# Giovannibriglia/ContinuousBayesianNetwork

Hardware: NVIDIA B200
Metric: posterior queries/sec (batched VE) (higher is better)
Workload: dtype f32

## Files before the change

continuousbayesiannetwork_b200/_native.py:

```python
from __future__ import annotations

import ctypes as C
import os
from typing import Dict, Sequence

PKG = os.path.dirname(os.path.abspath(__file__))
LIB_PATH = os.path.join(PKG, "libcbn_b200.so")

MAX_FAMILY_VARS = 12
MAX_CARD = 255
UNSEEN = 255
MAX_CONTRACT_DIMS = 24
MAX_CONTRACT_INPUTS = 16
MAX_GATHER_TABLES = 16
MAX_EVIDENCE_PTRS = 64
GATHER_MAX_CT = 8

OK, ERR_INVALID, ERR_CUDA, ERR_NOMEM, ERR_UNSUPPORTED = 0, -1, -2, -3, -4


class NativeLibraryMissing(ImportError):
    pass


# ... 96 lines not shown
    "cbn_cpt_from_counts": (C.c_int, [_P, _P, C.POINTER(Family), C.c_int32, C.c_longlong, _P, _P, _P]),
    "cbn_cpt_from_plan": (C.c_int, [_P, _P, _P, C.c_longlong, _P, _P, _P]),
    "cbn_cpt_from_plan_dev": (C.c_int, [_P, _P, _P, _P, _P, _P, _P]),
    "cbn_mle_from_counts": (C.c_int, [_P, _P, C.POINTER(Family), C.POINTER(_P), C.c_longlong, _P, _P, _P]),
    "cbn_get_prob_f32": (C.c_int, [_P, _P, C.POINTER(Family), C.POINTER(_P), _P, C.c_int64, C.c_int32, _P,
                                   C.c_int64, _P, _P]),
    "cbn_factor_contract": (C.c_int, [_P, C.POINTER(Contract), _P]),
    "cbn_factor_rescale": (C.c_int, [_P, _P, C.c_longlong, C.c_int32, C.c_int32, _P]),
    "cbn_ve_plan_create_gather": (C.c_int, [_P, C.c_int32, C.POINTER(C.c_int32), C.c_int32, C.POINTER(GatherTable),
                                            C.c_int32, C.c_int32, _P, C.POINTER(_P)]),
    "cbn_ve_plan_create_rows": (C.c_int, [_P, C.c_int32, C.POINTER(C.c_int32), C.c_int32, C.POINTER(RowInput), C.c_int32,
                                          C.POINTER(RowStep), C.c_int32, C.c_int32, _P, C.POINTER(_P)]),
    "cbn_ve_plan_destroy": (None, [_P]),
    "cbn_ve_plan_fuse": (C.c_int, [_P, C.POINTER(_P), C.c_int32, _P, C.POINTER(_P)]),
    "cbn_ve_plan_set_static_evidence": (C.c_int, [_P, C.c_int32]),
    "cbn_ve_plan_outputs": (C.c_int, [_P]),
    "cbn_ve_run_codes_multi": (C.c_int, [_P, _P, _P, C.c_int64, C.c_int64, C.POINTER(_P), _P]),
    "cbn_ve_run_codes": (C.c_int, [_P, _P, _P, C.c_int64, C.c_int64, _P, _P]),
    "cbn_ve_run_f32": (C.c_int, [_P, _P, C.POINTER(_P), C.POINTER(_P), C.c_int64, _P, _P]),
    "cbn_ve_run_codes_map": (C.c_int, [_P, _P, _P, C.c_int64, C.c_int64, _P, _P, _P]),
    "cbn_ve_run_f32_map": (C.c_int, [_P, _P, C.POINTER(_P), C.POINTER(_P), C.c_int64, _P, _P, _P]),
    "cbn_ve_run_codes_log_evidence": (C.c_int, [_P, _P, _P, C.c_int64, C.c_int64, _P, _P]),
    "cbn_loglik_plan_create": (C.c_int, [_P, C.POINTER(Family), C.c_int32, C.c_int32, _P, _P, C.POINTER(_P)]),
    "cbn_loglik_plan_destroy": (None, [_P]),
    "cbn_loglik_run": (C.c_int, [_P, _P, _P, C.c_int64, C.c_int64, _P, C.c_int32, _P]),
    "cbn_loglik_plan_tables": (C.c_int, [_P]),
    "cbn_factor_contract_max": (C.c_int, [_P, C.POINTER(Contract), _P, _P]),
    "cbn_mpe_plan_create": (C.c_int, [_P, C.c_int32, C.POINTER(C.c_int32), C.c_int32, C.POINTER(MpeStep), C.c_int32, _P,
                                      C.POINTER(_P)]),
    "cbn_mpe_plan_destroy": (None, [_P]),
# ... 112 lines not shown
```

continuousbayesiannetwork_b200/csrc/common.cuh:

```cuda
#pragma once
#include <cuda_runtime.h>
#include <stdint.h>
#include <stdio.h>
#include <stdarg.h>
#include <string>
#include <vector>

#include "cbn_b200.h"

struct cbn_ctx {
  int device = 0;
  int sm_count = 148;
  size_t smem_optin = 0;
  std::string err;
  cudaStream_t io_stream[2] = {nullptr, nullptr};
  cudaEvent_t io_event[2] = {nullptr, nullptr};
  void* io_dev_in[2] = {nullptr, nullptr};
  void* io_dev_out[2] = {nullptr, nullptr};
  void* io_pin_in[2] = {nullptr, nullptr};
  void* io_pin_out[2] = {nullptr, nullptr};
  size_t io_in_bytes = 0, io_out_bytes = 0;
  cudaMemPool_t pool = nullptr;
};

// ... 140 lines not shown
  asm volatile("ld.global.nc.L1::no_allocate.v8.f32 {%0,%1,%2,%3,%4,%5,%6,%7}, [%8];"
               : "=f"(v[0]), "=f"(v[1]), "=f"(v[2]), "=f"(v[3]), "=f"(v[4]), "=f"(v[5]), "=f"(v[6]), "=f"(v[7])
               : "l"(p));
}

__device__ __forceinline__ void st_f256_hint(float* p, const float* v, uint64_t pol) {
  asm volatile("st.global.L2::cache_hint.v8.f32 [%0], {%1,%2,%3,%4,%5,%6,%7,%8}, %9;" ::"l"(p), "f"(v[0]), "f"(v[1]), "f"(v[2]),
               "f"(v[3]), "f"(v[4]), "f"(v[5]), "f"(v[6]), "f"(v[7]), "l"(pol)
               : "memory");
}
__device__ __forceinline__ void ld_na_f256_hint(const float* p, float* v, uint64_t pol) {
  asm volatile("ld.global.nc.L1::no_allocate.L2::cache_hint.v8.f32 {%0,%1,%2,%3,%4,%5,%6,%7}, [%8], %9;"
               : "=f"(v[0]), "=f"(v[1]), "=f"(v[2]), "=f"(v[3]), "=f"(v[4]), "=f"(v[5]), "=f"(v[6]), "=f"(v[7])
               : "l"(p), "l"(pol));
}
__device__ __forceinline__ void bulk_g2s_hint(void* dst, const void* src, uint32_t bytes, uint64_t* bar, uint64_t pol) {
  asm volatile("cp.async.bulk.shared::cluster.global.mbarrier::complete_tx::bytes.L2::cache_hint [%0], [%1], %2, [%3], %4;" ::"r"(smem_u32(dst)),
               "l"(src), "r"(bytes), "r"(smem_u32(bar)), "l"(pol)
               : "memory");
}
```

continuousbayesiannetwork_b200/csrc/ve.cu:

```cuda
#include <stdlib.h>
#include <string.h>

#include <algorithm>
#include <new>

#include "common.cuh"

namespace {
struct ContractMagic { unsigned long long m[CBN_MAX_CONTRACT_DIMS]; int sh[CBN_MAX_CONTRACT_DIMS]; };

__device__ __forceinline__ float lse_pair(float a, float b) {
  const float NEG_INF = __int_as_float(0xff800000);
  const float hi = fmaxf(a, b), lo = fminf(a, b);
  return (hi == NEG_INF) ? NEG_INF : hi + log1pf(expf(lo - hi));
}

template <bool FAST, bool LOG, bool MAX = false>
__global__ void __launch_bounds__(256) contract_kernel(const __grid_constant__ cbn_contract d, const __grid_constant__ ContractMagic mg,
                                                       long long n_out, uint8_t* __restrict__ amax) {
  for (long long o = (long long)blockIdx.x * blockDim.x + threadIdx.x; o < n_out;
       o += (long long)gridDim.x * blockDim.x) {
    long long base[CBN_MAX_CONTRACT_INPUTS];
#pragma unroll
    for (int k = 0; k < CBN_MAX_CONTRACT_INPUTS; ++k) base[k] = 0;
// ... 328 lines not shown
  int n_out = 1;
  unsigned normalize_mask = 1;
  int log_space = 0;
  std::vector<int> ev_cards;
  std::vector<GTable> h_tables;
  int kind = 0;
  int rows_n_inputs = 0, rows_n_steps = 0, rows_temp_floats = 0, rows_flags = 0;
  void* d_row_inputs = nullptr;
  void* d_row_steps = nullptr;
  void* d_row_offsets = nullptr;
  int rows_off_ints = 0;
  size_t rows_thread_smem = 0;
  bool rows_per_thread = false;
  float* d_inter = nullptr;
  int interleaved = 0;
  unsigned char* d_blob = nullptr;
  size_t blob_bytes = 0;
  size_t desc_bytes = 0;
  int staged = 0;
  long long table_bytes = 0;
  int static_evidence = 0;
  mutable int occ[4] = {0, 0, 0, 0};
  mutable size_t occ_smem[4] = {0, 0, 0, 0};
};

namespace {
struct EvPtrs {
  const float* col[CBN_MAX_EVIDENCE_PTRS];
  const float* dom[CBN_MAX_EVIDENCE_PTRS];
  int card[CBN_MAX_EVIDENCE_PTRS];
// ... 46 lines not shown
  } else {
#pragma unroll
    for (int t = 0; t < CT; ++t) v[t] = src[t];
  }
}

template <int CT>
__device__ __forceinline__ void load_slice_l2(const float* __restrict__ src, float (&v)[CT]) {
  if constexpr (CT == 8) {
    ld_na_f256(src, v);
  } else if constexpr (CT == 4) {
    const float4 a = ld_nc_f128(reinterpret_cast<const float4*>(src));
    v[0] = a.x; v[1] = a.y; v[2] = a.z; v[3] = a.w;
  } else {
    load_slice<CT>(src, v);
  }
}

__device__ __forceinline__ void pdl_trigger() { asm volatile("griddepcontrol.launch_dependents;" ::: "memory"); }
__device__ __forceinline__ void pdl_wait() { asm volatile("griddepcontrol.wait;" ::: "memory"); }

template <int CT>
__device__ __forceinline__ void finish_rows4(float (&p)[4][CT], uint32_t bad, bool normalize, int64_t quad,
                                             int64_t n_rows, float* __restrict__ out, uint64_t st_pol = 0, bool log_space = false) {
  pdl_wait();
  if (log_space) {
#pragma unroll
    for (int r = 0; r < 4; ++r) {
      float m = p[r][0];
#pragma unroll
// ... 225 lines not shown
#pragma unroll
        for (int t = 0; t < CT; ++t) p[r][t] = lg ? p[r][t] + s : p[r][t] * s;
      }
    }
  }
  if (cur >= 0) finish_any4<CT, LOGEV>(p, bad, (outs.normalize_mask >> cur) & 1u, quad, n_rows, outs, cur, st_pol);
}

__device__ __forceinline__ void stage_blob(const unsigned char* __restrict__ blob, int blob_bytes, unsigned char* smem) {
  const uint4* src = reinterpret_cast<const uint4*>(blob);
  uint4* dst = reinterpret_cast<uint4*>(smem);
  for (int i = threadIdx.x; i < (blob_bytes >> 4); i += blockDim.x) dst[i] = __ldg(src + i);
  __syncthreads();
}

template <int CT, int NOUT, typename Loader>
__device__ __forceinline__ void gather_inter_rows4(const GTable& T, const float* __restrict__ base, const Loader& L,
                                                   int64_t quad, int64_t n_rows, const GatherOuts& outs, uint64_t st_pol = 0,
                                                   uint64_t ld_pol = 0) {
  constexpr int W = CT * NOUT;
  uint32_t i0 = 0, i1 = 0, i2 = 0, i3 = 0, any = 0, bad = 0;
  const int mode = T.flags >> GT_MODE_SHIFT;
  const int ne = T.n_ev;
  const uint32_t tm = ((quad << 2) + 4 <= n_rows) ? 0xffffffffu : ((1u << (8 * int(n_rows - (quad << 2)))) - 1u);
  if (mode == 0) {
    uint32_t acc = 0;
#pragma unroll 4
    for (int j = 0; j < ne; ++j) {
      const uint32_t w = L.load4(T.slot[j], quad) & tm;
      any |= w;
      acc += w * (uint32_t)T.stride[j];
    }
    i0 = acc & 0xffu; i1 = (acc >> 8) & 0xffu; i2 = (acc >> 16) & 0xffu; i3 = acc >> 24;
  } else if (mode == 1) {
    uint32_t accE = 0, accO = 0;
// ... 18 lines not shown
  const uint32_t lim = (uint32_t)T.n_cells - W;
  if (any & 0x80808080u) {
    const uint4 e = exact_index4(T, L, quad, lim, &bad);
    i0 = e.x; i1 = e.y; i2 = e.z; i3 = e.w;
    bad &= tm == 0xffffffffu ? 0xfu : ((1u << int(n_rows - (quad << 2))) - 1u);
  }
  i0 = min(i0, lim); i1 = min(i1, lim); i2 = min(i2, lim); i3 = min(i3, lim);
  const uint32_t idx[4] = {i0, i1, i2, i3};
  float v[4][W];
  if (T.smem_off >= 0) {
#pragma unroll
    for (int r = 0; r < 4; ++r) load_slice<W>(base + idx[r], v[r]);
  } else if (W == 8 && ld_pol) {
#pragma unroll
    for (int r = 0; r < 4; ++r) ld_na_f256_hint(base + idx[r], v[r], ld_pol);
  } else {
#pragma unroll
    for (int r = 0; r < 4; ++r) load_slice_l2<W>(base + idx[r], v[r]);
  }
#pragma unroll
  for (int o = 0; o < NOUT; ++o) {
    float p[4][CT];
#pragma unroll
    for (int r = 0; r < 4; ++r)
#pragma unroll
      for (int t = 0; t < CT; ++t) p[r][t] = v[r][o * CT + t];
    finish_rows4<CT>(p, bad, false, quad, n_rows, outs.out[o], st_pol);
  }
}

template <int CT, int NOUT>
__global__ void __launch_bounds__(GATHER_TPB) gather_inter_kernel(const unsigned char* __restrict__ blob, int blob_bytes,
                                                                  int desc_bytes, const uint8_t* __restrict__ ev, int64_t ld,
                                                                  int64_t n_rows, int early_ev, const __grid_constant__ GatherOuts outs) {
  extern __shared__ __align__(16) unsigned char smem_raw[];
  pdl_trigger();
  stage_blob(blob, blob_bytes, smem_raw);
  if (!early_ev) pdl_wait();
  const GTable& T = *reinterpret_cast<const GTable*>(smem_raw);
  const float* base = T.smem_off >= 0 ? reinterpret_cast<const float*>(smem_raw + desc_bytes) + T.smem_off : T.data;
  CodeLoader L{ev, ld};
  const int64_t nquads = (n_rows + 3) >> 2;
  for (int64_t q = int64_t(blockIdx.x) * blockDim.x + threadIdx.x; q < nquads; q += int64_t(gridDim.x) * blockDim.x)
    gather_inter_rows4<CT, NOUT>(T, base, L, q, n_rows, outs);
}

constexpr int GT_MAX_QPT = 2;
constexpr int GT_TILE_ROWS_MAX = 4 * GATHER_TPB * GT_MAX_QPT;
constexpr int GT_MAX_COLS = 16;
constexpr int GT_MAX_STAGES = 4;

struct TileCols {
  int n;
  uint8_t slot[GT_MAX_COLS];
};
template <int TILE_ROWS>
struct TileLoader {
  const unsigned char* stage;
  int64_t quad0;
  __device__ __forceinline__ uint32_t load4(int col, int64_t quad) const {
    return *reinterpret_cast<const uint32_t*>(stage + col * TILE_ROWS + (int(quad - quad0) << 2));
  }
};

template <int CT, int NOUT, int GT_QPT, bool LOGEV = false>
__global__ void __launch_bounds__(GATHER_TPB) gather_tiles_kernel(const unsigned char* __restrict__ blob, int blob_bytes,
                                                                  int desc_bytes, int n_tables, const __grid_constant__ TileCols cols,
                                                                  int n_stages, int hints, const uint8_t* __restrict__ ev, int64_t ld,
                                                                  int64_t n_rows, int early_ev, const __grid_constant__ GatherOuts outs) {
  constexpr int GT_TILE_ROWS = 4 * GATHER_TPB * GT_QPT;
  extern __shared__ __align__(128) unsigned char smem_raw[];
  __shared__ __align__(8) uint64_t full[GT_MAX_STAGES], empty[GT_MAX_STAGES];
  pdl_trigger();
  stage_blob(blob, blob_bytes, smem_raw);
  if (!early_ev) pdl_wait();
  GTable* st = reinterpret_cast<GTable*>(smem_raw);
  for (int i = threadIdx.x; i < n_tables * GATHER_MAX_TABLE_EV; i += blockDim.x) {
    GTable& T = st[i / GATHER_MAX_TABLE_EV];
    const int j = i % GATHER_MAX_TABLE_EV;
    if (j < T.n_ev) {
// ... 42 lines not shown
        if (i > 0) mbar_wait(&empty[(i - 1) % n_stages], uint32_t((i - 1) / n_stages) & 1u);
        issue(nxt);
      }
    }
    mbar_wait(&full[s], round & 1u);
    const int64_t tile = int64_t(blockIdx.x) + i * gridDim.x;
    const int64_t q0 = tile * (GT_TILE_ROWS / 4);
    TileLoader<GT_TILE_ROWS> L{stages + size_t(s) * stage_bytes, q0};
#pragma unroll 1
    for (int qq = 0; qq < GT_QPT; ++qq) {
      const int64_t q = q0 + qq * GATHER_TPB + threadIdx.x;
      if (q < nquads) {
        if constexpr (NOUT >= 2) {
          const GTable& T = st[0];
          const float* base = T.smem_off >= 0 ? pool + T.smem_off : T.data;
          gather_inter_rows4<CT, NOUT>(T, base, L, q, n_rows, outs, st_pol, ld_pol);
        } else {
          gather_rows4<CT, TileLoader<GT_TILE_ROWS>, LOGEV>(st, n_tables, pool, L, q, n_rows, outs, st_pol, ld_pol);
        }
      }
    }
    __syncwarp();
    if (lane == 0) mbar_arrive(&empty[s]);
  }
}

constexpr int gather_min_blocks(int ct) { return ct <= 2 ? 6 : (ct <= 4 ? 5 : 3); }

template <int CT, bool LOGEV = false>
__global__ void __launch_bounds__(GATHER_TPB, gather_min_blocks(LOGEV && CT == 2 ? 3 : CT)) gather_codes_kernel(
    const unsigned char* __restrict__ blob, int blob_bytes, int desc_bytes, int n_tables, const uint8_t* __restrict__ ev,
// ... 167 lines not shown
  if (rc) { cbn_ve_plan_destroy(p); return rc; }
  *out = p;
  return CBN_OK;
}

extern "C" int cbn_ve_plan_fuse(cbn_ctx* ctx, const cbn_ve_plan* const* plans, int32_t n_plans, cbn_stream stream,
                                cbn_ve_plan** out) {
  cudaStream_t cs = (cudaStream_t)stream;
  if (!ctx) return cbn_fail(nullptr, CBN_ERR_INVALID, "cbn_ve_plan_fuse: ctx is NULL");
  if (!plans || !out || n_plans < 1) return cbn_fail(ctx, CBN_ERR_INVALID, "cbn_ve_plan_fuse: bad argument");
  DeviceGuard g(ctx->device);
  cbn_ve_plan* p = new (std::nothrow) cbn_ve_plan();
  if (!p) return cbn_fail(ctx, CBN_ERR_NOMEM, "out of host memory");
  p->device = ctx->device;
  p->n_out = 0; p->normalize_mask = 0;
  for (int i = 0; i < n_plans; ++i) {
    const cbn_ve_plan* q = plans[i];
    if (!q) { delete p; return cbn_fail(ctx, CBN_ERR_INVALID, "cbn_ve_plan_fuse: plan %d is NULL", i); }
    if (q->kind != 0) { delete p; return cbn_fail(ctx, CBN_ERR_INVALID, "cbn_ve_plan_fuse: per-row plans cannot be fused"); }
    if (i == 0) { p->n_evidence = q->n_evidence; p->ev_cards = q->ev_cards; p->card_t = q->card_t; p->log_space = q->log_space; }
    if (q->ev_cards != p->ev_cards || q->card_t != p->card_t || q->log_space != p->log_space) {
      delete p;
      return cbn_fail(ctx, CBN_ERR_INVALID, "cbn_ve_plan_fuse: plans must share the evidence list, the target cardinality and the number space");
    }
    for (int o = 0; o < q->n_out; ++o) {
      if (p->n_out >= GATHER_MAX_OUT) { delete p; return cbn_fail(ctx, CBN_ERR_UNSUPPORTED, "cbn_ve_plan_fuse: at most %d targets per launch", GATHER_MAX_OUT); }
      for (const GTable& t : q->h_tables)
        if (t.out_id == o) { GTable c = t; c.out_id = p->n_out; p->h_tables.push_back(c); }
      if ((q->normalize_mask >> o) & 1u) p->normalize_mask |= 1u << p->n_out;
      p->n_out += 1;
    }
  }
  {
    const int n_out = p->n_out, ct = p->card_t, w = n_out * ct;
    bool ok = n_out >= 2 && ct >= 2 && (int)p->h_tables.size() == n_out && p->normalize_mask == 0 && ct <= GATHER_MAX_CT &&
              (w == 4 || w == 6 || w == 8);
    for (int k = 0; ok && k < n_out; ++k) {
      const GTable& t = p->h_tables[k];
      ok = (t.flags & GT_HAS_TARGET) && t.out_id == k && (k == 0 || same_index(t, p->h_tables[0])) &&
           (long long)t.n_cells * n_out <= 0x7fffffffll;
    }
    if (ok) {
      const long long n_cfg = p->h_tables[0].n_cells / ct;
      cudaError_t e = cudaMalloc((void**)&p->d_inter, size_t(n_cfg) * w * sizeof(float));
      for (int k = 0; e == cudaSuccess && k < n_out; ++k)
        e = cudaMemcpy2DAsync(p->d_inter + k * ct, size_t(w) * sizeof(float), p->h_tables[k].data, size_t(ct) * sizeof(float),
                              size_t(ct) * sizeof(float), size_t(n_cfg), cudaMemcpyDeviceToDevice, cs);
      if (e != cudaSuccess) { cbn_ve_plan_destroy(p); return cbn_fail(ctx, CBN_ERR_CUDA, "interleave: %s", cudaGetErrorString(e)); }
      GTable t = p->h_tables[0];
      t.data = p->d_inter;
      t.n_cells = (int)(n_cfg * w);
      for (int j = 0; j < t.n_ev; ++j) t.stride[j] *= n_out;
      p->h_tables.assign(1, t);
      p->interleaved = n_out;
    }
  }
  int rc = finalize_plan(ctx, p, cs);
  if (rc) { cbn_ve_plan_destroy(p); return rc; }
  *out = p;
  return CBN_OK;
}

extern "C" int cbn_ve_plan_set_static_evidence(cbn_ve_plan* plan, int32_t on) {
  if (!plan) return CBN_ERR_INVALID;
  plan->static_evidence = on ? 1 : 0;
  return CBN_OK;
}

extern "C" int cbn_ve_plan_outputs(const cbn_ve_plan* plan) { return plan ? plan->n_out : 0; }

extern "C" void cbn_ve_plan_destroy(cbn_ve_plan* p) {
  if (!p) return;
  DeviceGuard g(p->device);
  if (p->d_blob) cudaFree(p->d_blob);
// ... 54 lines not shown
int launch_f32(cbn_ctx* ctx, const cbn_ve_plan* p, const EvPtrs& evp, size_t dom_floats, int64_t n_rows, const GatherOuts& outs,
               cudaStream_t s) {
  static bool attr_set[64] = {};
  if (!attr_set[ctx->device & 63]) {
    CBN_CUDA(ctx, cudaFuncSetAttribute(gather_f32_kernel<CT>, cudaFuncAttributeMaxDynamicSharedMemorySize, 160 * 1024));
    attr_set[ctx->device & 63] = true;
  }
  size_t smem = p->blob_bytes + dom_floats * 4;
  int per_sm = (int)std::max<size_t>(1, std::min<size_t>(4, (200 * 1024) / (smem + 1024)));
  gather_f32_kernel<CT><<<gather_blocks(ctx, n_rows, per_sm), GATHER_TPB, smem, s>>>(
      p->d_blob, (int)p->blob_bytes, (int)p->desc_bytes, p->n_tables, evp, p->n_evidence, n_rows, outs);
  CBN_CHECK_LAUNCH(ctx);
  return CBN_OK;
}

template <int CT, int NOUT>
int launch_inter(cbn_ctx* ctx, const cbn_ve_plan* p, const uint8_t* ev, int64_t ld, int64_t n_rows, const GatherOuts& outs,
                 cudaStream_t s) {
  static bool attr_set[64] = {};
  if (!attr_set[ctx->device & 63]) {
    CBN_CUDA(ctx, cudaFuncSetAttribute(gather_inter_kernel<CT, NOUT>, cudaFuncAttributeMaxDynamicSharedMemorySize, 100 * 1024));
    attr_set[ctx->device & 63] = true;
  }
  if (p->occ[0] == 0 || p->occ_smem[0] != p->blob_bytes) {
    int occ = 1;
    CBN_CUDA(ctx, cudaOccupancyMaxActiveBlocksPerMultiprocessor(&occ, gather_inter_kernel<CT, NOUT>, GATHER_TPB, p->blob_bytes));
    p->occ[0] = std::max(occ, 1); p->occ_smem[0] = p->blob_bytes;
  }
  const int per_sm = p->occ[0];
  CBN_CUDA(ctx, launch_pdl(gather_inter_kernel<CT, NOUT>, gather_blocks(ctx, n_rows, per_sm), GATHER_TPB, p->blob_bytes, s,
                           p->d_blob, (int)p->blob_bytes, (int)p->desc_bytes, ev, ld, n_rows, p->static_evidence, outs));
  return CBN_OK;
}

template <int CT, int NOUT, int QPT, bool LOGEV = false>
int launch_tiles_q(cbn_ctx* ctx, const cbn_ve_plan* p, const uint8_t* ev, int64_t ld, int64_t n_rows, const GatherOuts& outs,
                   cudaStream_t s) {
  TileCols cols{};
  for (const GTable& t : p->h_tables)
    for (int j = 0; j < t.n_ev; ++j) {
      int c = 0;
      while (c < cols.n && cols.slot[c] != t.slot[j]) ++c;
      if (c == cols.n) cols.slot[cols.n++] = t.slot[j];
    }
  constexpr int GT_TILE_ROWS = 4 * GATHER_TPB * QPT;
  const size_t blob_pad = (p->blob_bytes + 127) & ~size_t(127);
  const size_t stage_bytes = size_t(cols.n) * GT_TILE_ROWS;
  int n_stages = 3;
  static int stages_env = -1;
  if (stages_env < 0) { const char* e = getenv("CBN_GATHER_STAGES"); stages_env = e ? atoi(e) : 0; }
  if (stages_env >= 2 && stages_env <= GT_MAX_STAGES) n_stages = stages_env;
  while (n_stages > 2 && blob_pad + n_stages * stage_bytes > 56 * 1024) --n_stages;
  const int hints = 7;
  const size_t smem = blob_pad + n_stages * stage_bytes;
  static bool attr_set[64] = {};
  if (!attr_set[ctx->device & 63]) {
    CBN_CUDA(ctx, cudaFuncSetAttribute(gather_tiles_kernel<CT, NOUT, QPT, LOGEV>, cudaFuncAttributeMaxDynamicSharedMemorySize, 160 * 1024));
    attr_set[ctx->device & 63] = true;
  }
  const int slot = LOGEV ? 3 : 1;
  if (p->occ[slot] == 0 || p->occ_smem[slot] != smem) {
    int occ = 1;
    CBN_CUDA(ctx, cudaOccupancyMaxActiveBlocksPerMultiprocessor(&occ, gather_tiles_kernel<CT, NOUT, QPT, LOGEV>, GATHER_TPB, smem));
    p->occ[slot] = std::max(occ, 1); p->occ_smem[slot] = smem;
  }
  const int64_t n_tiles = (n_rows + GT_TILE_ROWS - 1) / GT_TILE_ROWS;
  const int per_sm = p->occ[slot];
  const int blocks = (int)balanced_grid(n_tiles, int64_t(ctx->sm_count) * per_sm);
  CBN_CUDA(ctx, launch_pdl(gather_tiles_kernel<CT, NOUT, QPT, LOGEV>, blocks, GATHER_TPB, smem, s, p->d_blob, (int)p->blob_bytes,
                           (int)p->desc_bytes, p->n_tables, cols, n_stages, hints, ev, ld, n_rows, p->static_evidence, outs));
  return CBN_OK;
}

template <int CT, int NOUT>
int launch_tiles(cbn_ctx* ctx, const cbn_ve_plan* p, const uint8_t* ev, int64_t ld, int64_t n_rows, const GatherOuts& outs,
                 cudaStream_t s) {
  if constexpr (NOUT >= 2) {
    static int qpt_env = -1;
    if (qpt_env < 0) { const char* e = getenv("CBN_GATHER_QPT"); qpt_env = e ? atoi(e) : 0; }
    const int64_t big_tiles = n_rows / (4 * GATHER_TPB * GT_MAX_QPT);
    const bool two = qpt_env ? qpt_env == 2 : big_tiles >= int64_t(ctx->sm_count) * 4 * 10;
    if (two) return launch_tiles_q<CT, NOUT, 2>(ctx, p, ev, ld, n_rows, outs, s);
  }
  return launch_tiles_q<CT, NOUT, 1>(ctx, p, ev, ld, n_rows, outs, s);
}

bool use_tiles(const cbn_ve_plan* p, int64_t n_rows, bool force = false) {
  static int mode = -2;
  if (mode == -2) { const char* e = getenv("CBN_GATHER_TILES"); mode = e ? atoi(e) : -1; }
  if (mode == 0 || p->card_t > GATHER_MAX_CT || p->n_evidence < 1) return false;
  std::vector<char> seen(256, 0);
  int n = 0;
  for (const GTable& t : p->h_tables)
    for (int j = 0; j < t.n_ev; ++j)
      if (!seen[t.slot[j]]) { seen[t.slot[j]] = 1; ++n; }
  if (n < 1 || n > GT_MAX_COLS) return false;
  if (((p->blob_bytes + 127) & ~size_t(127)) + 2 * size_t(n) * GT_TILE_ROWS_MAX > 150 * 1024) return false;
  if (!p->staged && p->table_bytes >= (4ll << 20) && n_rows >= (int64_t(1) << 18)) return true;
  return force || mode == 1 || n_rows >= (int64_t(1) << 21);
}

int ve_run_codes_impl(cbn_ctx* ctx, const cbn_ve_plan* plan, const uint8_t* ev_codes, int64_t ld, int64_t n_rows,
                      const GatherOuts& outs, cudaStream_t s, bool force_tiles = false) {
  const bool tiles = use_tiles(plan, n_rows, force_tiles);
  if (plan->interleaved) {
    const int key = plan->card_t * 10 + plan->interleaved;
    if (tiles) switch (key) {
      case 22: return launch_tiles<2, 2>(ctx, plan, ev_codes, ld, n_rows, outs, s);
      case 23: return launch_tiles<2, 3>(ctx, plan, ev_codes, ld, n_rows, outs, s);
      case 24: return launch_tiles<2, 4>(ctx, plan, ev_codes, ld, n_rows, outs, s);
      case 32: return launch_tiles<3, 2>(ctx, plan, ev_codes, ld, n_rows, outs, s);
      case 42: return launch_tiles<4, 2>(ctx, plan, ev_codes, ld, n_rows, outs, s);
      default: break;
    }
    switch (key) {
      case 22: return launch_inter<2, 2>(ctx, plan, ev_codes, ld, n_rows, outs, s);
      case 23: return launch_inter<2, 3>(ctx, plan, ev_codes, ld, n_rows, outs, s);
      case 24: return launch_inter<2, 4>(ctx, plan, ev_codes, ld, n_rows, outs, s);
      case 32: return launch_inter<3, 2>(ctx, plan, ev_codes, ld, n_rows, outs, s);
      case 42: return launch_inter<4, 2>(ctx, plan, ev_codes, ld, n_rows, outs, s);
      default: return cbn_fail(ctx, CBN_ERR_UNSUPPORTED, "internal: interleaved plan %d x %d", plan->card_t, plan->interleaved);
// ... 1045 lines not shown
```

continuousbayesiannetwork_b200/ve.py:

```python
from __future__ import annotations

import ctypes as C
from dataclasses import dataclass, field
from typing import Dict, List, Optional, Sequence, Tuple

import torch

from . import _native as N


class PlanTooLarge(NotImplementedError):
    pass


def _prod(it) -> int:
    p = 1
    for x in it:
        p *= int(x)
    return p


@dataclass
class Factor:
    scope: List[int]
# ... 13 lines not shown
    n_steps: int = 0
    max_table_cells: int = 0
    contraction_madds: int = 0
    final_tables: List[Tuple[Tuple[int, ...], int]] = field(default_factory=list)
    support_unchecked: bool = False
    per_row_hidden: int = 0
    per_row_madds: int = 0
    per_row_slice_cells: int = 0
    contraction_gpu_ms: float = 0.0
    relevant_evidence: List[int] = field(default_factory=list)


class QueryPlan:

    def __init__(self, tables_owner, target: int, evidence: List[int], card_t: int, finals: List[Factor],
                 normalize: bool, stats: PlanStats, log_space: bool = False):
        self.owner = tables_owner
        self.ctx = tables_owner.ctx
        self.device = tables_owner.device
        self.target = target
        self.evidence = list(evidence)
        self.card_t = card_t
        self.finals = finals
        self.normalize = normalize
        self.log_space = bool(log_space)
        self.stats = stats
        self.handle = None
        cards = tables_owner.cards
        slot = {v: i for i, v in enumerate(self.evidence)}
        arr = (N.GatherTable * len(finals))()
        for k, f in enumerate(finals):
            has_t = bool(f.scope) and f.scope[-1] == target
            ev_scope = f.scope[:-1] if has_t else f.scope
            g = arr[k]
            g.data = f.tensor.data_ptr()
            g.n_cells = f.tensor.numel()
            g.n_ev = len(ev_scope)
            g.has_target = 1 if has_t else 0
            stride = card_t if has_t else 1
            for j in range(len(ev_scope) - 1, -1, -1):
                g.ev_slot[j] = slot[ev_scope[j]]
                g.ev_stride[j] = stride
                stride *= cards[ev_scope[j]]
        ev_cards = (C.c_int32 * max(len(self.evidence), 1))(*[cards[v] for v in self.evidence])
        h = C.c_void_p()
        N.check(N.lib().cbn_ve_plan_create_gather(self.ctx.handle, len(self.evidence), ev_cards, card_t, arr, len(finals),
                                                  (N.GATHER_NORMALIZE if normalize else 0) | (N.GATHER_LOG_SPACE if log_space else 0),
                                                  N.stream_ptr(self.device), C.byref(h)), self.ctx.handle)
        self.handle = h

    def __del__(self):
        try:
            if self.handle is not None:
                N.lib().cbn_ve_plan_destroy(self.handle)
                self.handle = None
        except Exception:
            pass

    def algorithmic_bytes_per_row(self) -> int:
        return len(self.stats.relevant_evidence) + 4 * self.card_t

    def run_codes(self, ev_codes: torch.Tensor, n_rows: int, out: Optional[torch.Tensor] = None) -> torch.Tensor:
        assert ev_codes.dtype == torch.uint8 and ev_codes.is_cuda
        if out is None:
# ... 595 lines not shown
            stats.final_tables = [(tuple(f.scope), f.size(cards)) for f in finals]
            stats.per_row_slice_cells = sum(int(f.size(cards) // max(1, _prod(cards[v] for v in f.scope if v in Eset))) for f in finals)
            plan = self._row_plan(T, E, finals, left, stats, dry)
            if dry:
                return stats
            stats.contraction_gpu_ms = self._drain_events()
            self._cache[key] = plan
            return plan
        finals = self._merge_finals(finals, sort_scope, stats, dry, T)
        stats.final_tables = [(tuple(f.scope), f.size(cards)) for f in finals]
        if dry:
            return stats
        normalize = True
        with_t = [f for f in finals if f.scope and f.scope[-1] == T]
        log_tables = self.log_space
        if len(finals) == 1 and len(with_t) == 1:
            finals = [self._contract(finals, finals[0].scope, None, dry, normalize_last=True)]
            normalize = False
            log_tables = False
        if not with_t:
            raise RuntimeError("internal: no final factor mentions the target")
        stats.contraction_gpu_ms = self._drain_events()
        plan = QueryPlan(t, T, E, cards[T], finals, normalize, stats, log_space=log_tables)
        self._cache[key] = plan
        return plan

    def compile_evidence(self, evidence_names: Sequence[str], dry: bool = False):
        if not self.log_space or self.rescale:
            return self._evidence_child().compile_evidence(evidence_names, dry=dry)
        t = self.t
        cards = t.cards
        E = self._evidence_ids(evidence_names)
        key = tuple(E)
        if not dry:
            self._drop_stale_plans()
            if key in self._ev_cache:
                return self._ev_cache[key]
            self.compile_evidence(evidence_names, dry=True)
# ... 368 lines not shown
```

include/cbn_b200.h:

```cpp
#ifndef CBN_B200_H
#define CBN_B200_H

#include <stdint.h>

#ifdef __cplusplus
extern "C" {
#endif

#if defined(__GNUC__)
#define CBN_API __attribute__((visibility("default")))
#else
#define CBN_API
#endif

#define CBN_ABI_VERSION 2
#define CBN_MAX_FAMILY_VARS 12
#define CBN_MAX_CARD 255
#define CBN_UNSEEN 255
#define CBN_MAX_CONTRACT_DIMS 24
#define CBN_MAX_CONTRACT_INPUTS 16
#define CBN_MAX_GATHER_TABLES 16
#define CBN_MAX_EVIDENCE_PTRS 64

typedef enum cbn_status {
// ... 90 lines not shown
  int32_t n_ev;
  int32_t ev_slot[CBN_MAX_CONTRACT_DIMS];
  int32_t ev_stride[CBN_MAX_CONTRACT_DIMS];
  int32_t has_target;
} cbn_gather_table;

#define CBN_GATHER_NORMALIZE 1
#define CBN_GATHER_LOG_SPACE 2
CBN_API int cbn_ve_plan_create_gather(cbn_ctx* ctx, int32_t n_evidence, const int32_t* ev_cards, int32_t card_t,
                              const cbn_gather_table* tables, int32_t n_tables, int32_t normalize,
                              cbn_stream stream, cbn_ve_plan** out);
CBN_API void cbn_ve_plan_destroy(cbn_ve_plan* plan);
CBN_API int cbn_ve_plan_fuse(cbn_ctx* ctx, const cbn_ve_plan* const* plans, int32_t n_plans, cbn_stream stream,
                     cbn_ve_plan** out);
CBN_API int cbn_ve_plan_set_static_evidence(cbn_ve_plan* plan, int32_t on);
CBN_API int cbn_ve_plan_outputs(const cbn_ve_plan* plan);

#define CBN_ROWS_LOG_SPACE 1
typedef struct cbn_row_input {
  const float* data;
  int64_t n_cells;
  int32_t n_ev;
  int32_t ev_slot[CBN_MAX_CONTRACT_DIMS];
  int32_t ev_stride[CBN_MAX_CONTRACT_DIMS];
} cbn_row_input;
typedef struct cbn_row_step {
  int32_t out_size;
  int32_t sum_card;
  int32_t n_in;
  int32_t in_id[CBN_MAX_CONTRACT_INPUTS];
// ... 68 lines not shown
```

Measured before the change: 471.5 billion.

## Pack binary-target posteriors into one float per config for fused gather

For binary targets, each normalized (p0,p1) pair is encoded as a single signed float that stores the smaller probability, with the sign marking which state is larger. Fused interleaved tables then hold one float per target instead of two, which halves the gather footprint and load width. Decoding rebuilds the larger value as 1 minus the smaller one. The original tables are rewritten in canonical form so outputs match the compact path, which costs a little precision on the larger probability. The tiles path also gets a shared-memory carveout hint and an occupancy cap.

Result: faster. 480.9 billion, median of 6 (+2.0%).

```diff
diff --git a/continuousbayesiannetwork_b200/_native.py b/continuousbayesiannetwork_b200/_native.py
--- a/continuousbayesiannetwork_b200/_native.py
+++ b/continuousbayesiannetwork_b200/_native.py
@@ -134,6 +134,8 @@
     "cbn_ve_plan_destroy": (None, [_P]),
     "cbn_ve_plan_fuse": (C.c_int, [_P, C.POINTER(_P), C.c_int32, _P, C.POINTER(_P)]),
     "cbn_ve_plan_set_static_evidence": (C.c_int, [_P, C.c_int32]),
+    "cbn_ve_binary_canonical": (C.c_int, [_P, _P, _P, C.c_longlong, _P]),
+    "cbn_ve_plan_set_binary_compact": (C.c_int, [_P, _P]),
     "cbn_ve_plan_outputs": (C.c_int, [_P]),
     "cbn_ve_run_codes_multi": (C.c_int, [_P, _P, _P, C.c_int64, C.c_int64, C.POINTER(_P), _P]),
     "cbn_ve_run_codes": (C.c_int, [_P, _P, _P, C.c_int64, C.c_int64, _P, _P]),
diff --git a/continuousbayesiannetwork_b200/csrc/common.cuh b/continuousbayesiannetwork_b200/csrc/common.cuh
--- a/continuousbayesiannetwork_b200/csrc/common.cuh
+++ b/continuousbayesiannetwork_b200/csrc/common.cuh
@@ -178,6 +178,14 @@
                : "=f"(v[0]), "=f"(v[1]), "=f"(v[2]), "=f"(v[3]), "=f"(v[4]), "=f"(v[5]), "=f"(v[6]), "=f"(v[7])
                : "l"(p), "l"(pol));
 }
+__device__ __forceinline__ void ld_na_f128_hint(const float* p, float* v, uint64_t pol) {
+  asm volatile("ld.global.nc.L1::no_allocate.L2::cache_hint.v4.f32 {%0,%1,%2,%3}, [%4], %5;"
+               : "=f"(v[0]), "=f"(v[1]), "=f"(v[2]), "=f"(v[3])
+               : "l"(p), "l"(pol));
+}
+__device__ __forceinline__ void ld_na_f64_hint(const float* p, float* v, uint64_t pol) {
+  asm volatile("ld.global.nc.L1::no_allocate.L2::cache_hint.v2.f32 {%0,%1}, [%2], %3;" : "=f"(v[0]), "=f"(v[1]) : "l"(p), "l"(pol));
+}
 __device__ __forceinline__ void bulk_g2s_hint(void* dst, const void* src, uint32_t bytes, uint64_t* bar, uint64_t pol) {
   asm volatile("cp.async.bulk.shared::cluster.global.mbarrier::complete_tx::bytes.L2::cache_hint [%0], [%1], %2, [%3], %4;" ::"r"(smem_u32(dst)),
                "l"(src), "r"(bytes), "r"(smem_u32(bar)), "l"(pol)
diff --git a/continuousbayesiannetwork_b200/csrc/ve.cu b/continuousbayesiannetwork_b200/csrc/ve.cu
--- a/continuousbayesiannetwork_b200/csrc/ve.cu
+++ b/continuousbayesiannetwork_b200/csrc/ve.cu
@@ -366,6 +366,8 @@
   bool rows_per_thread = false;
   float* d_inter = nullptr;
   int interleaved = 0;
+  int inter_compact = 0;
+  const float* compact = nullptr;
   unsigned char* d_blob = nullptr;
   size_t blob_bytes = 0;
   size_t desc_bytes = 0;
@@ -442,6 +444,31 @@
     v[0] = a.x; v[1] = a.y; v[2] = a.z; v[3] = a.w;
   } else {
     load_slice<CT>(src, v);
+  }
+}
+
+__device__ __forceinline__ float binary_compact_encode(float p0, float p1) {
+  if (!(p0 > 0.0f) && !(p1 > 0.0f)) return __int_as_float(0x7f800000);
+  return p1 > p0 ? -p0 : p1;
+}
+__device__ __forceinline__ void binary_compact_decode(float c, float& p0, float& p1) {
+  const float small = fabsf(c);
+  const bool dead = small > 1.0f;
+  const float big = dead ? 0.0f : __fsub_rn(1.0f, small);
+  const float lo = dead ? 0.0f : small;
+  const bool one = signbit(c);
+  p0 = one ? lo : big;
+  p1 = one ? big : lo;
+}
+
+__global__ void __launch_bounds__(256) binary_canonical_kernel(float2* __restrict__ pairs, float* __restrict__ compact, long long n_cfg) {
+  for (long long i = (long long)blockIdx.x * blockDim.x + threadIdx.x; i < n_cfg; i += (long long)gridDim.x * blockDim.x) {
+    const float2 q = pairs[i];
+    const float s = binary_compact_encode(q.x, q.y);
+    float2 d;
+    binary_compact_decode(s, d.x, d.y);
+    compact[i] = s;
+    pairs[i] = d;
   }
 }
 
@@ -697,11 +724,12 @@
   __syncthreads();
 }
 
-template <int CT, int NOUT, typename Loader>
+template <int CT, int NOUT, bool COMPACT, typename Loader>
 __device__ __forceinline__ void gather_inter_rows4(const GTable& T, const float* __restrict__ base, const Loader& L,
                                                    int64_t quad, int64_t n_rows, const GatherOuts& outs, uint64_t st_pol = 0,
                                                    uint64_t ld_pol = 0) {
-  constexpr int W = CT * NOUT;
+  static_assert(!COMPACT || (CT == 2 && NOUT >= 2 && NOUT <= 4), "compact tables hold 2 to 4 binary targets");
+  constexpr int W = COMPACT ? (NOUT == 2 ? 2 : 4) : CT * NOUT;
   uint32_t i0 = 0, i1 = 0, i2 = 0, i3 = 0, any = 0, bad = 0;
   const int mode = T.flags >> GT_MODE_SHIFT;
   const int ne = T.n_ev;
@@ -750,6 +778,12 @@
   } else if (W == 8 && ld_pol) {
 #pragma unroll
     for (int r = 0; r < 4; ++r) ld_na_f256_hint(base + idx[r], v[r], ld_pol);
+  } else if (COMPACT && ld_pol) {
+#pragma unroll
+    for (int r = 0; r < 4; ++r) {
+      if constexpr (W == 4) ld_na_f128_hint(base + idx[r], v[r], ld_pol);
+      else ld_na_f64_hint(base + idx[r], v[r], ld_pol);
+    }
   } else {
 #pragma unroll
     for (int r = 0; r < 4; ++r) load_slice_l2<W>(base + idx[r], v[r]);
@@ -758,14 +792,19 @@
   for (int o = 0; o < NOUT; ++o) {
     float p[4][CT];
 #pragma unroll
-    for (int r = 0; r < 4; ++r)
-#pragma unroll
-      for (int t = 0; t < CT; ++t) p[r][t] = v[r][o * CT + t];
+    for (int r = 0; r < 4; ++r) {
+      if constexpr (COMPACT) {
+        binary_compact_decode(v[r][o], p[r][0], p[r][1 % CT]);
+      } else {
+#pragma unroll
+        for (int t = 0; t < CT; ++t) p[r][t] = v[r][o * CT + t];
+      }
+    }
     finish_rows4<CT>(p, bad, false, quad, n_rows, outs.out[o], st_pol);
   }
 }
 
-template <int CT, int NOUT>
+template <int CT, int NOUT, bool COMPACT = false>
 __global__ void __launch_bounds__(GATHER_TPB) gather_inter_kernel(const unsigned char* __restrict__ blob, int blob_bytes,
                                                                   int desc_bytes, const uint8_t* __restrict__ ev, int64_t ld,
                                                                   int64_t n_rows, int early_ev, const __grid_constant__ GatherOuts outs) {
@@ -778,7 +817,7 @@
   CodeLoader L{ev, ld};
   const int64_t nquads = (n_rows + 3) >> 2;
   for (int64_t q = int64_t(blockIdx.x) * blockDim.x + threadIdx.x; q < nquads; q += int64_t(gridDim.x) * blockDim.x)
-    gather_inter_rows4<CT, NOUT>(T, base, L, q, n_rows, outs);
+    gather_inter_rows4<CT, NOUT, COMPACT>(T, base, L, q, n_rows, outs);
 }
 
 constexpr int GT_MAX_QPT = 2;
@@ -799,7 +838,7 @@
   }
 };
 
-template <int CT, int NOUT, int GT_QPT, bool LOGEV = false>
+template <int CT, int NOUT, int GT_QPT, bool LOGEV = false, bool COMPACT = false>
 __global__ void __launch_bounds__(GATHER_TPB) gather_tiles_kernel(const unsigned char* __restrict__ blob, int blob_bytes,
                                                                   int desc_bytes, int n_tables, const __grid_constant__ TileCols cols,
                                                                   int n_stages, int hints, const uint8_t* __restrict__ ev, int64_t ld,
@@ -872,7 +911,7 @@
         if constexpr (NOUT >= 2) {
           const GTable& T = st[0];
           const float* base = T.smem_off >= 0 ? pool + T.smem_off : T.data;
-          gather_inter_rows4<CT, NOUT>(T, base, L, q, n_rows, outs, st_pol, ld_pol);
+          gather_inter_rows4<CT, NOUT, COMPACT>(T, base, L, q, n_rows, outs, st_pol, ld_pol);
         } else {
           gather_rows4<CT, TileLoader<GT_TILE_ROWS>, LOGEV>(st, n_tables, pool, L, q, n_rows, outs, st_pol, ld_pol);
         }
@@ -1070,6 +1109,7 @@
   if (!p) return cbn_fail(ctx, CBN_ERR_NOMEM, "out of host memory");
   p->device = ctx->device;
   p->n_out = 0; p->normalize_mask = 0;
+  std::vector<const float*> compacts;
   for (int i = 0; i < n_plans; ++i) {
     const cbn_ve_plan* q = plans[i];
     if (!q) { delete p; return cbn_fail(ctx, CBN_ERR_INVALID, "cbn_ve_plan_fuse: plan %d is NULL", i); }
@@ -1079,6 +1119,7 @@
       delete p;
       return cbn_fail(ctx, CBN_ERR_INVALID, "cbn_ve_plan_fuse: plans must share the evidence list, the target cardinality and the number space");
     }
+    if (q->compact && q->n_out == 1 && (int)compacts.size() == p->n_out) compacts.push_back(q->compact);
     for (int o = 0; o < q->n_out; ++o) {
       if (p->n_out >= GATHER_MAX_OUT) { delete p; return cbn_fail(ctx, CBN_ERR_UNSUPPORTED, "cbn_ve_plan_fuse: at most %d targets per launch", GATHER_MAX_OUT); }
       for (const GTable& t : q->h_tables)
@@ -1097,23 +1138,51 @@
            (long long)t.n_cells * n_out <= 0x7fffffffll;
     }
     if (ok) {
+      const bool packed = ct == 2 && (int)compacts.size() == n_out;
+      const int wr = packed ? (n_out == 2 ? 2 : 4) : w;
       const long long n_cfg = p->h_tables[0].n_cells / ct;
-      cudaError_t e = cudaMalloc((void**)&p->d_inter, size_t(n_cfg) * w * sizeof(float));
+      cudaError_t e = cudaMalloc((void**)&p->d_inter, size_t(n_cfg) * wr * sizeof(float));
+      if (e == cudaSuccess && packed && wr != n_out) e = cudaMemsetAsync(p->d_inter, 0, size_t(n_cfg) * wr * sizeof(float), cs);
       for (int k = 0; e == cudaSuccess && k < n_out; ++k)
-        e = cudaMemcpy2DAsync(p->d_inter + k * ct, size_t(w) * sizeof(float), p->h_tables[k].data, size_t(ct) * sizeof(float),
-                              size_t(ct) * sizeof(float), size_t(n_cfg), cudaMemcpyDeviceToDevice, cs);
+        e = packed ? cudaMemcpy2DAsync(p->d_inter + k, size_t(wr) * sizeof(float), compacts[k], sizeof(float), sizeof(float),
+                                    size_t(n_cfg), cudaMemcpyDeviceToDevice, cs)
+                : cudaMemcpy2DAsync(p->d_inter + k * ct, size_t(w) * sizeof(float), p->h_tables[k].data, size_t(ct) * sizeof(float),
+                                    size_t(ct) * sizeof(float), size_t(n_cfg), cudaMemcpyDeviceToDevice, cs);
       if (e != cudaSuccess) { cbn_ve_plan_destroy(p); return cbn_fail(ctx, CBN_ERR_CUDA, "interleave: %s", cudaGetErrorString(e)); }
       GTable t = p->h_tables[0];
       t.data = p->d_inter;
-      t.n_cells = (int)(n_cfg * w);
-      for (int j = 0; j < t.n_ev; ++j) t.stride[j] *= n_out;
+      t.n_cells = (int)(n_cfg * wr);
+      for (int j = 0; j < t.n_ev; ++j) t.stride[j] = packed ? t.stride[j] / ct * wr : t.stride[j] * n_out;
       p->h_tables.assign(1, t);
       p->interleaved = n_out;
+      p->inter_compact = packed ? 1 : 0;
     }
   }
   int rc = finalize_plan(ctx, p, cs);
   if (rc) { cbn_ve_plan_destroy(p); return rc; }
   *out = p;
+  return CBN_OK;
+}
+
+extern "C" int cbn_ve_binary_canonical(cbn_ctx* ctx, float* table, float* compact_out, long long n_cfg, cbn_stream stream) {
+  if (!ctx) return cbn_fail(nullptr, CBN_ERR_INVALID, "cbn_ve_binary_canonical: ctx is NULL");
+  if (n_cfg < 0 || (n_cfg > 0 && (!table || !compact_out)))
+    return cbn_fail(ctx, CBN_ERR_INVALID, "cbn_ve_binary_canonical: bad argument");
+  if (n_cfg == 0) return CBN_OK;
+  if (!is_aligned(table, 8)) return cbn_fail(ctx, CBN_ERR_INVALID, "cbn_ve_binary_canonical: table must be 8-byte aligned");
+  DeviceGuard g(ctx->device);
+  const int blocks = (int)std::min<long long>((n_cfg + 255) / 256, (long long)ctx->sm_count * 16);
+  binary_canonical_kernel<<<blocks, 256, 0, (cudaStream_t)stream>>>(reinterpret_cast<float2*>(table), compact_out, n_cfg);
+  CBN_CHECK_LAUNCH(ctx);
+  return CBN_OK;
+}
+
+extern "C" int cbn_ve_plan_set_binary_compact(cbn_ve_plan* plan, const float* compact) {
+  if (!plan) return CBN_ERR_INVALID;
+  if (compact && (plan->kind != 0 || plan->card_t != 2 || plan->n_out != 1 || plan->h_tables.size() != 1 ||
+                !(plan->h_tables[0].flags & GT_HAS_TARGET) || plan->normalize_mask != 0 || plan->log_space))
+    return CBN_ERR_INVALID;
+  plan->compact = compact;
   return CBN_OK;
 }
 
@@ -1198,26 +1267,26 @@
   return CBN_OK;
 }
 
-template <int CT, int NOUT>
+template <int CT, int NOUT, bool COMPACT = false>
 int launch_inter(cbn_ctx* ctx, const cbn_ve_plan* p, const uint8_t* ev, int64_t ld, int64_t n_rows, const GatherOuts& outs,
                  cudaStream_t s) {
   static bool attr_set[64] = {};
   if (!attr_set[ctx->device & 63]) {
-    CBN_CUDA(ctx, cudaFuncSetAttribute(gather_inter_kernel<CT, NOUT>, cudaFuncAttributeMaxDynamicSharedMemorySize, 100 * 1024));
+    CBN_CUDA(ctx, cudaFuncSetAttribute(gather_inter_kernel<CT, NOUT, COMPACT>, cudaFuncAttributeMaxDynamicSharedMemorySize, 100 * 1024));
     attr_set[ctx->device & 63] = true;
   }
   if (p->occ[0] == 0 || p->occ_smem[0] != p->blob_bytes) {
     int occ = 1;
-    CBN_CUDA(ctx, cudaOccupancyMaxActiveBlocksPerMultiprocessor(&occ, gather_inter_kernel<CT, NOUT>, GATHER_TPB, p->blob_bytes));
+    CBN_CUDA(ctx, cudaOccupancyMaxActiveBlocksPerMultiprocessor(&occ, gather_inter_kernel<CT, NOUT, COMPACT>, GATHER_TPB, p->blob_bytes));
     p->occ[0] = std::max(occ, 1); p->occ_smem[0] = p->blob_bytes;
   }
   const int per_sm = p->occ[0];
-  CBN_CUDA(ctx, launch_pdl(gather_inter_kernel<CT, NOUT>, gather_blocks(ctx, n_rows, per_sm), GATHER_TPB, p->blob_bytes, s,
+  CBN_CUDA(ctx, launch_pdl(gather_inter_kernel<CT, NOUT, COMPACT>, gather_blocks(ctx, n_rows, per_sm), GATHER_TPB, p->blob_bytes, s,
                            p->d_blob, (int)p->blob_bytes, (int)p->desc_bytes, ev, ld, n_rows, p->static_evidence, outs));
   return CBN_OK;
 }
 
-template <int CT, int NOUT, int QPT, bool LOGEV = false>
+template <int CT, int NOUT, int QPT, bool LOGEV = false, bool COMPACT = false>
 int launch_tiles_q(cbn_ctx* ctx, const cbn_ve_plan* p, const uint8_t* ev, int64_t ld, int64_t n_rows, const GatherOuts& outs,
                    cudaStream_t s) {
   TileCols cols{};
@@ -1239,24 +1308,28 @@
   const size_t smem = blob_pad + n_stages * stage_bytes;
   static bool attr_set[64] = {};
   if (!attr_set[ctx->device & 63]) {
-    CBN_CUDA(ctx, cudaFuncSetAttribute(gather_tiles_kernel<CT, NOUT, QPT, LOGEV>, cudaFuncAttributeMaxDynamicSharedMemorySize, 160 * 1024));
+    CBN_CUDA(ctx, cudaFuncSetAttribute(gather_tiles_kernel<CT, NOUT, QPT, LOGEV, COMPACT>, cudaFuncAttributeMaxDynamicSharedMemorySize, 160 * 1024));
+    if constexpr (COMPACT) {
+      CBN_CUDA(ctx, cudaFuncSetAttribute(gather_tiles_kernel<CT, NOUT, QPT, LOGEV, COMPACT>, cudaFuncAttributePreferredSharedMemoryCarveout, 71));
+    }
     attr_set[ctx->device & 63] = true;
   }
   const int slot = LOGEV ? 3 : 1;
   if (p->occ[slot] == 0 || p->occ_smem[slot] != smem) {
     int occ = 1;
-    CBN_CUDA(ctx, cudaOccupancyMaxActiveBlocksPerMultiprocessor(&occ, gather_tiles_kernel<CT, NOUT, QPT, LOGEV>, GATHER_TPB, smem));
+    CBN_CUDA(ctx, cudaOccupancyMaxActiveBlocksPerMultiprocessor(&occ, gather_tiles_kernel<CT, NOUT, QPT, LOGEV, COMPACT>, GATHER_TPB, smem));
+    if constexpr (COMPACT) occ = std::min(occ, int((164 * 1024) / (smem + 1024)));
     p->occ[slot] = std::max(occ, 1); p->occ_smem[slot] = smem;
   }
   const int64_t n_tiles = (n_rows + GT_TILE_ROWS - 1) / GT_TILE_ROWS;
   const int per_sm = p->occ[slot];
   const int blocks = (int)balanced_grid(n_tiles, int64_t(ctx->sm_count) * per_sm);
-  CBN_CUDA(ctx, launch_pdl(gather_tiles_kernel<CT, NOUT, QPT, LOGEV>, blocks, GATHER_TPB, smem, s, p->d_blob, (int)p->blob_bytes,
+  CBN_CUDA(ctx, launch_pdl(gather_tiles_kernel<CT, NOUT, QPT, LOGEV, COMPACT>, blocks, GATHER_TPB, smem, s, p->d_blob, (int)p->blob_bytes,
                            (int)p->desc_bytes, p->n_tables, cols, n_stages, hints, ev, ld, n_rows, p->static_evidence, outs));
   return CBN_OK;
 }
 
-template <int CT, int NOUT>
+template <int CT, int NOUT, bool COMPACT = false>
 int launch_tiles(cbn_ctx* ctx, const cbn_ve_plan* p, const uint8_t* ev, int64_t ld, int64_t n_rows, const GatherOuts& outs,
                  cudaStream_t s) {
   if constexpr (NOUT >= 2) {
@@ -1264,9 +1337,9 @@
     if (qpt_env < 0) { const char* e = getenv("CBN_GATHER_QPT"); qpt_env = e ? atoi(e) : 0; }
     const int64_t big_tiles = n_rows / (4 * GATHER_TPB * GT_MAX_QPT);
     const bool two = qpt_env ? qpt_env == 2 : big_tiles >= int64_t(ctx->sm_count) * 4 * 10;
-    if (two) return launch_tiles_q<CT, NOUT, 2>(ctx, p, ev, ld, n_rows, outs, s);
-  }
-  return launch_tiles_q<CT, NOUT, 1>(ctx, p, ev, ld, n_rows, outs, s);
+    if (two) return launch_tiles_q<CT, NOUT, 2, false, COMPACT>(ctx, p, ev, ld, n_rows, outs, s);
+  }
+  return launch_tiles_q<CT, NOUT, 1, false, COMPACT>(ctx, p, ev, ld, n_rows, outs, s);
 }
 
 bool use_tiles(const cbn_ve_plan* p, int64_t n_rows, bool force = false) {
@@ -1289,6 +1362,20 @@
   const bool tiles = use_tiles(plan, n_rows, force_tiles);
   if (plan->interleaved) {
     const int key = plan->card_t * 10 + plan->interleaved;
+    if (plan->inter_compact) {
+      if (tiles) switch (key) {
+        case 22: return launch_tiles<2, 2, true>(ctx, plan, ev_codes, ld, n_rows, outs, s);
+        case 23: return launch_tiles<2, 3, true>(ctx, plan, ev_codes, ld, n_rows, outs, s);
+        case 24: return launch_tiles<2, 4, true>(ctx, plan, ev_codes, ld, n_rows, outs, s);
+        default: break;
+      }
+      switch (key) {
+        case 22: return launch_inter<2, 2, true>(ctx, plan, ev_codes, ld, n_rows, outs, s);
+        case 23: return launch_inter<2, 3, true>(ctx, plan, ev_codes, ld, n_rows, outs, s);
+        case 24: return launch_inter<2, 4, true>(ctx, plan, ev_codes, ld, n_rows, outs, s);
+        default: return cbn_fail(ctx, CBN_ERR_UNSUPPORTED, "internal: compact plan of %d targets", plan->interleaved);
+      }
+    }
     if (tiles) switch (key) {
       case 22: return launch_tiles<2, 2>(ctx, plan, ev_codes, ld, n_rows, outs, s);
       case 23: return launch_tiles<2, 3>(ctx, plan, ev_codes, ld, n_rows, outs, s);
diff --git a/continuousbayesiannetwork_b200/ve.py b/continuousbayesiannetwork_b200/ve.py
--- a/continuousbayesiannetwork_b200/ve.py
+++ b/continuousbayesiannetwork_b200/ve.py
@@ -51,7 +51,7 @@
 class QueryPlan:
 
     def __init__(self, tables_owner, target: int, evidence: List[int], card_t: int, finals: List[Factor],
-                 normalize: bool, stats: PlanStats, log_space: bool = False):
+                 normalize: bool, stats: PlanStats, log_space: bool = False, compact: Optional[torch.Tensor] = None):
         self.owner = tables_owner
         self.ctx = tables_owner.ctx
         self.device = tables_owner.device
@@ -59,6 +59,7 @@
         self.evidence = list(evidence)
         self.card_t = card_t
         self.finals = finals
+        self.compact = compact
         self.normalize = normalize
         self.log_space = bool(log_space)
         self.stats = stats
@@ -85,6 +86,8 @@
                                                   (N.GATHER_NORMALIZE if normalize else 0) | (N.GATHER_LOG_SPACE if log_space else 0),
                                                   N.stream_ptr(self.device), C.byref(h)), self.ctx.handle)
         self.handle = h
+        if compact is not None:
+            N.check(N.lib().cbn_ve_plan_set_binary_compact(h, compact.data_ptr()), self.ctx.handle)
 
     def __del__(self):
         try:
@@ -710,14 +713,20 @@
         normalize = True
         with_t = [f for f in finals if f.scope and f.scope[-1] == T]
         log_tables = self.log_space
+        compact = None
         if len(finals) == 1 and len(with_t) == 1:
             finals = [self._contract(finals, finals[0].scope, None, dry, normalize_last=True)]
             normalize = False
             log_tables = False
+            if cards[T] == 2:
+                tab = finals[0].tensor
+                compact = torch.empty(max(tab.numel() // 2, 1), dtype=torch.float32, device=t.device)
+                N.check(N.lib().cbn_ve_binary_canonical(t.ctx.handle, tab.data_ptr(), compact.data_ptr(), tab.numel() // 2,
+                                                        N.stream_ptr(t.device)), t.ctx.handle)
         if not with_t:
             raise RuntimeError("internal: no final factor mentions the target")
         stats.contraction_gpu_ms = self._drain_events()
-        plan = QueryPlan(t, T, E, cards[T], finals, normalize, stats, log_space=log_tables)
+        plan = QueryPlan(t, T, E, cards[T], finals, normalize, stats, log_space=log_tables, compact=compact)
         self._cache[key] = plan
         return plan
 
diff --git a/include/cbn_b200.h b/include/cbn_b200.h
--- a/include/cbn_b200.h
+++ b/include/cbn_b200.h
@@ -128,6 +128,8 @@
 CBN_API int cbn_ve_plan_fuse(cbn_ctx* ctx, const cbn_ve_plan* const* plans, int32_t n_plans, cbn_stream stream,
                      cbn_ve_plan** out);
 CBN_API int cbn_ve_plan_set_static_evidence(cbn_ve_plan* plan, int32_t on);
+CBN_API int cbn_ve_binary_canonical(cbn_ctx* ctx, float* table, float* compact_out, long long n_cfg, cbn_stream stream);
+CBN_API int cbn_ve_plan_set_binary_compact(cbn_ve_plan* plan, const float* compact);
 CBN_API int cbn_ve_plan_outputs(const cbn_ve_plan* plan);
 
 #define CBN_ROWS_LOG_SPACE 1
```
